# datatypevoid/babble

Measured on AMD Instinct MI355X. Metric: consensus-ordered events/sec at N=256 peers (1 GPU and 8-GPU batched sims), higher is better.
Workload: dtype int32

## Files before the change

### babble_amd/csrc/hgx_api.cpp

```cpp
#include <algorithm>
#include <array>
#include <chrono>
#include <cstdio>
#include <cstring>
#include <mutex>
#include <tuple>
#include <set>
#include <new>
#include <cstdlib>
#include <string>
#include <thread>
#include <vector>

#include "hgx.h"
#include "hgx_bodies.h"
#include "hgx_diff.h"
#include "hgx_engine.h"
#include "hgx_wire_plan.h"

namespace {

struct Block {
    int32_t rr;
    int64_t first;
// ... 2518 lines not shown
    if (x == y) return 1;
    if (!known_div(c, x) || !known_div(c, y)) return 0;
    DeviceGuard dg(c);
    if (ensure_mirror(c) || !same_graph(c, x, y)) return 0;
    std::vector<int32_t> la(c->n), fd(c->n);
    if (c->eng.get_coords(x, la.data(), fd.data()) != hipSuccess) return 0;
    return la[c->creator[(size_t)y] % c->n] >= c->index32[(size_t)y] ? 1 : 0;
}
int32_t hgx_self_ancestor(hgx_ctx* c, int64_t x, int64_t y) {
    if (x == y) return 1;
    if (!c || x < 0 || y < 0 || x >= c->E || y >= c->E) return 0;
    DeviceGuard dg(c);
    if (ensure_mirror(c)) return 0;
    return (c->creator[(size_t)x] == c->creator[(size_t)y] && c->index32[(size_t)x] >= c->index32[(size_t)y]) ? 1 : 0;
}
int32_t hgx_see(hgx_ctx* c, int64_t x, int64_t y) { return hgx_ancestor(c, x, y); }
int32_t hgx_strongly_see(hgx_ctx* c, int64_t x, int64_t y) {
    if (!known_div(c, x) || !known_div(c, y)) return 0;
    DeviceGuard dg(c);
    if (ensure_mirror(c) || !same_graph(c, x, y)) return 0;
    std::vector<int32_t> lx(c->n), fx(c->n), ly(c->n), fy(c->n);
    if (c->eng.get_coords(x, lx.data(), fx.data()) != hipSuccess) return 0;
    if (c->eng.get_coords(y, ly.data(), fy.data()) != hipSuccess) return 0;
    int cnt = 0;
    for (int i = 0; i < c->n; i++) cnt += lx[i] >= fy[i];
    return cnt >= c->sm ? 1 : 0;
}
int64_t hgx_oldest_self_ancestor_to_see(hgx_ctx* c, int64_t x, int64_t y) {
    if (!known_div(c, x) || !known_div(c, y)) return -1;
    DeviceGuard dg(c);
    if (ensure_chains(c) || !same_graph(c, x, y)) return -1;
    std::vector<int32_t> la(c->n), fd(c->n);
    if (c->eng.get_coords(y, la.data(), fd.data()) != hipSuccess) return -1;
    const int cx = c->creator[(size_t)x];
    const int32_t a = fd[cx % c->n];
    if (a <= c->index32[(size_t)x]) return c->chain_gids[cx][(size_t)(a - c->chain_base[cx])];
    return -1;
}
int32_t hgx_round(hgx_ctx* c, int64_t x) {
    if (!c) return -1;
    DeviceGuard dg(c);
    if (ensure_rounds(c)) return -1;
    return round_of(c, x);
}
int32_t hgx_witness(hgx_ctx* c, int64_t x) {
    if (!c) return 0;
    DeviceGuard dg(c);
    if (ensure_rounds(c) || ensure_mirror(c)) return 0;
    return witness_of(c, x);
}

int32_t hgx_phase_times(hgx_ctx* c, double* out, int32_t cap) {
    if (!c || !out) return 0;
    const int32_t m = std::min<int32_t>(cap, 27);
    double v[27] = {c->eng.phase_ms[0], c->eng.phase_ms[1], c->eng.phase_ms[2], c->eng.phase_ms[3],
                    (double)c->eng.la_sweeps, (double)c->eng.R, (double)c->eng.compact,
                    (double)c->eng.la_rows, c->eng.last_rebuild ? 1.0 : 0.0, (double)c->rh.r_lo,
                    c->eng.la_wave_used ? 1.0 : 0.0, (double)c->eng.la_wave_fallbacks,
                    (double)(c->eng.la_wave_used ? c->eng.la_wave_segs : 0), (double)c->eng.round_p_runs,
                    (double)c->eng.round_p_fallbacks, (double)c->eng.round_p_ovf,
                    (double)c->eng.round_p_fail_round, (double)c->eng.round_p_fail_chain,
                    (double)c->eng.round_g_runs, c->eng.la_small_used ? 1.0 : 0.0,
                    c->eng.la_verified ? 1.0 : 0.0, (double)c->eng.sort_seg_runs, (double)c->eng.pipe_used,
                    c->host_ms[0], c->host_ms[1], c->host_ms[2], c->host_ms[3]};
    for (int32_t i = 0; i < m; i++) out[i] = v[i];
    return m;
}

static const char* kKernelNames[hgx::K_NUM] = {"layout", "la_sweep", "fd_build", "round_gather", "round_search",
                                              "fame", "threshold", "round_received", "cts_median", "order_sort"};

int32_t hgx_kernel_stats(hgx_ctx* c, int32_t k, char* name, int32_t name_cap, double* ms, int64_t* launches,
                         double* bytes) {
    if (!c || k < 0 || k >= hgx::K_NUM) return HGX_ERR_INVALID;
    if (name && name_cap > 0) std::snprintf(name, (size_t)name_cap, "%s", kKernelNames[k]);
    const hgx::KernelStat& ks = c->eng.kstat[k];
    if (ms) *ms = (ks.timed > 0 && ks.timed < ks.launches) ? ks.ms * (double)ks.launches / (double)ks.timed : ks.ms;
    if (launches) *launches = c->eng.kstat[k].launches;
    if (bytes) *bytes = c->eng.kstat[k].bytes;
    return HGX_OK;
}

int32_t hgx_reset_stats(hgx_ctx* c) {
    if (!c) return HGX_ERR_INVALID;
    for (auto& s : c->eng.kstat) s = hgx::KernelStat();
    return HGX_OK;
}

int32_t hgx_set_coord_storage(hgx_ctx* c, int32_t mode) {
    if (!c || mode < 0 || mode > 1) return HGX_ERR_INVALID;
    each_shard(c, [&](hgx_ctx* x) { x->eng.force_coord32 = mode == 1; });
    return HGX_OK;
}

int32_t hgx_set_kernel_timing(hgx_ctx* c, int32_t on) {
    if (!c) return HGX_ERR_INVALID;
    each_shard(c, [&](hgx_ctx* x) { x->eng.time_mask = (uint32_t)on; });
    return HGX_OK;
}

int32_t hgx_set_fame_tally(hgx_ctx* c, int32_t mode) {
    if (!c || mode < 0 || mode > 2) return HGX_ERR_INVALID;
    each_shard(c, [&](hgx_ctx* x) { x->eng.fame_tally = mode; });
    return HGX_OK;
}

int32_t hgx_device_alloc(int32_t device, int64_t bytes, void** ptr) {
    if (!ptr || bytes < 0) return HGX_ERR_INVALID;
    *ptr = nullptr;
    int prev = -1;
    (void)hipGetDevice(&prev);
    if (hipSetDevice(device) != hipSuccess) return HGX_ERR_DEVICE;
    const hipError_t e = hipMalloc(ptr, (size_t)std::max<int64_t>(bytes, 1));
    if (prev >= 0 && prev != device) (void)hipSetDevice(prev);
    return e == hipSuccess ? HGX_OK : HGX_ERR_DEVICE;
}

// ... 144 lines not shown
        q->eng.la_segs_override = c->eng.la_segs_override;
        q->eng.la_small_override = c->eng.la_small_override;
        q->eng.round_kernel = c->eng.round_kernel;
        q->eng.round_pb_enabled = c->eng.round_pb_enabled;
        q->eng.sort_seg_enabled = c->eng.sort_seg_enabled;
        q->eng.cts_kernel = c->eng.cts_kernel;
        q->eng.incremental = c->eng.incremental;
        q->grp = nullptr;
        c->peers.push_back(q);
    }
    std::vector<hgx_ctx*> sh{c};
    sh.insert(sh.end(), c->peers.begin(), c->peers.end());
    for (int k = 0; k < W; k++) {
        g->eng[k] = &sh[k]->eng;
        sh[k]->eng.grp = g;
        sh[k]->eng.shard = k;
        sh[k]->shard_rank = k;
        sh[k]->shard_world = W;
        sh[k]->eng.shard_lo = g->c_split[k];
        sh[k]->eng.shard_hi = g->c_split[k + 1];
    }
    return ok(err);
}

int32_t hgx_set_shard_remote(hgx_ctx* c, int32_t on) {
    if (!c || !c->grp || on < 0 || on > 1) return HGX_ERR_INVALID;
    c->grp->force_remote = on != 0;
    return HGX_OK;
}

int32_t hgx_set_round_shards(hgx_ctx* c, int32_t shards) {
    if (!c || shards < 1 || shards > hgx::kMaxShards) return HGX_ERR_INVALID;
    if (shards == (c->grp ? c->grp->W : 1)) return HGX_OK;
    std::vector<int32_t> devs((size_t)shards, c->eng.dev);
    return setup_group(c, shards, devs.data(), nullptr);
}

hgx_ctx* hgx_create_sharded(int32_t n_participants, int64_t capacity_events, int32_t n_shards, const int32_t* devices,
                            hgx_error* err) {
    if (n_shards < 1 || n_shards > hgx::kMaxShards || !devices) {
        set_err(err, HGX_ERR_INVALID, "hgx_create_sharded: 1 to 8 shards, one device ordinal each");
        return nullptr;
    }
    hgx_ctx* c = hgx_create_batch(1, n_participants, capacity_events, devices[0], err);
    if (!c) return nullptr;
    if (setup_group(c, n_shards, devices, err) != HGX_OK) {
        hgx_destroy(c);
        return nullptr;
    }
    return c;
}

int32_t hgx_set_cts_kernel(hgx_ctx* c, int32_t mode) {
    if (!c || mode < 0 || mode > 2) return HGX_ERR_INVALID;
    each_shard(c, [&](hgx_ctx* x) { x->eng.cts_kernel = mode == 0 ? 1 : mode; });
    return HGX_OK;
}

int32_t hgx_set_commit_callback(hgx_ctx* c, hgx_commit_fn fn, void* user) {
    if (!c) return HGX_ERR_INVALID;
    c->commit_fn = fn;
    c->commit_user = user;
    return HGX_OK;
}

int32_t hgx_set_incremental(hgx_ctx* c, int32_t on) {
    if (!c || on < 0 || on > 1) return HGX_ERR_INVALID;
    each_shard(c, [&](hgx_ctx* x) { x->eng.incremental = on != 0; });
    return HGX_OK;
}

int32_t hgx_reserve_rounds(hgx_ctx* c, int32_t rounds) {
    if (!c || rounds < 1 || c->divided) return HGX_ERR_INVALID;
    int32_t rc = HGX_OK;
    each_shard(c, [&](hgx_ctx* x) {
        DeviceGuard dg(x);
        if (x->eng.reserve_rounds(rounds) != hipSuccess) rc = HGX_ERR_DEVICE;
        x->rounds_cached = x->recv_cached = false;
    });
    return rc;
}

}
```

### babble_amd/csrc/hgx_cts.hip

```cpp
#include <hip/hip_runtime.h>

#include <algorithm>
#include <climits>
#include <cstdint>

#include "hgx_device.h"
#include "hgx_kernels.h"

namespace hgx {

constexpr int kCpT = 8;
constexpr int kCpRing = 4;
constexpr int kCpMaxC = 4096;
constexpr int64_t kCtsRedo = (int64_t)0x8000000000000000ull;

struct CtsTileInfo {
    int32_t row[kCpT];
    int64_t ts[kCpT];
    int32_t tc, p0;
};

__device__ __forceinline__ void cp_lds_barrier() { asm volatile("s_waitcnt lgkmcnt(0)\n\ts_barrier" ::: "memory"); }
__device__ __forceinline__ void cp_order() { asm volatile("" ::: "memory"); }

// ... 209 lines not shown
        const int64_t res = (int64_t)(wave_select_kth<CPL>(v, ok, m / 2, whist[wave]) ^ 0x8000000000000000ull);
        if (lane == 0) p_cts[p] = res;
    }
}

template <int NPAD, typename CT>
static bool cts_pipe_launch(hipStream_t s, const DevArrays& a, int c_lo, int c_cnt, int C, int n, int64_t P,
                            int max_cnt) {
    constexpr int LD = kCpT + 1;
    const size_t lds = (((size_t)4 * C + (size_t)8 * c_cnt + 15) & ~(size_t)15) + (size_t)2 * NPAD * LD * 5;
    const void* f = (const void*)k_cts_pipe<NPAD, CT>;
    static int dev_cus[64] = {0};
    int dev = 0;
    if (hipGetDevice(&dev) != hipSuccess || dev < 0 || dev >= 64) return false;
    if (ensure_lds_limit(f, lds) != hipSuccess) return false;
    if (dev_cus[dev] == 0) {
        int cus = 0;
        if (hipDeviceGetAttribute(&cus, hipDeviceAttributeMultiprocessorCount, dev) != hipSuccess || cus <= 0)
            return false;
        dev_cus[dev] = cus;
    }
    int per_cu = 0;
    if (blocks_per_cu(f, 256, lds, &per_cu) != hipSuccess || per_cu < 1) return false;
    const int ntt = (max_cnt + kCpT - 1) / kCpT;
    const int64_t tiles = (int64_t)c_cnt * ntt;
    if (tiles <= 0) return true;
    if (tiles > 0x7FFFFFFF - (int64_t)dev_cus[dev] * per_cu) return false;
    const unsigned grid = (unsigned)std::min<int64_t>(tiles, (int64_t)dev_cus[dev] * per_cu);
    hipLaunchKernelGGL((k_cts_pipe<NPAD, CT>), dim3(grid), dim3(256), lds, s, a.fu, a.rcnt, a.p_rr, a.c_off, a.c_base,
                       a.WLAT, (const CT*)a.FDT, a.p_ts, a.p_cts, C, n, P, c_lo, c_cnt, ntt);
    hipLaunchKernelGGL((k_cts_redo<NPAD, CT>), dim3((max_cnt + 255) / 256, c_cnt), dim3(256), 0, s, a.fu, a.rcnt, a.p_rr,
                       a.c_off, a.c_base, a.WLAT, (const CT*)a.FDT, a.p_ts, a.p_cts, C, n, P, c_lo);
    return true;
}

template <typename CT>
static bool launch_cts_pipe_t(hipStream_t s, const DevArrays& a, int c_lo, int c_cnt, int C, int n, int64_t P,
                              int max_cnt) {
    if (n <= 64) return cts_pipe_launch<64, CT>(s, a, c_lo, c_cnt, C, n, P, max_cnt);
    if (n <= 128) return cts_pipe_launch<128, CT>(s, a, c_lo, c_cnt, C, n, P, max_cnt);
    if (n <= 256) return cts_pipe_launch<256, CT>(s, a, c_lo, c_cnt, C, n, P, max_cnt);
    return cts_pipe_launch<512, CT>(s, a, c_lo, c_cnt, C, n, P, max_cnt);
}

bool cts_pipe_ok(int n, int C) { return n > 32 && n <= 512 && C <= kCpMaxC; }

bool launch_cts_pipe(hipStream_t s, const DevArrays& a, int c_lo, int c_cnt, int C, int n, int64_t P, int max_cnt) {
    if (max_cnt <= 0 || c_cnt <= 0) return true;
    if (!cts_pipe_ok(n, C)) return false;
    return a.compact ? launch_cts_pipe_t<uint16_t>(s, a, c_lo, c_cnt, C, n, P, max_cnt)
                     : launch_cts_pipe_t<int32_t>(s, a, c_lo, c_cnt, C, n, P, max_cnt);
}

}
```

### babble_amd/csrc/hgx_engine.cpp

```cpp
#include "hgx_engine.h"

#include <algorithm>
#include <array>
#include <chrono>
#include <cstdio>
#include <cstdlib>
#include <cstring>
#include <functional>

namespace hgx {

#define HGX_TRY(x)                              \
    do {                                        \
        hipError_t _e = (x);                    \
        if (_e != hipSuccess) return _e;        \
    } while (0)

template <typename T>
hipError_t DBuf<T>::alloc(size_t count) {
    release();
    if (count == 0) count = 1;
    hipError_t e = hipMalloc((void**)&p, count * sizeof(T));
    if (e == hipSuccess) n = count; else p = nullptr;
    return e;
// ... 2019 lines not shown
    return find_order_end(out, nullptr);
}

hipError_t Engine::find_order_begin(const std::vector<uint8_t>& el, const std::vector<uint8_t>& famous,
                                    const std::vector<uint8_t>& ure, int32_t r0, int max_unrecv, OrderHost& out) {
    stage_out.clear();
    pend.clear();
    stage_used = 0;
    out = OrderHost();
    fo_m = 0;
    fo_cnt.assign(C, 0);
    if (R == 0 || E_div == 0 || max_unrecv == 0 || r0 >= R) return hipSuccess;
    DevArrays a = arrays();
    HGX_TRY(hipEventRecord(ph0, stream));
    const size_t o = (size_t)r0 * C;
    HGX_TRY(stage_h2d(elig.p, el.data(), (size_t)G * R));
    HGX_TRY(stage_h2d(fw.p + o, famous.data() + o, (size_t)R * C - o));
    HGX_TRY(stage_h2d(ur_empty.p, ure.data(), (size_t)G));
    HGX_TRY(stage_issue());
    if (WLAT.n < (size_t)R * C * n) {
        const size_t want = (size_t)R * C * n + (size_t)C * n;
        const size_t first = WLAT.n ? 0 : std::min((size_t)r_cap * C * n, (size_t)1 << 28);
        HGX_TRY(WLAT.alloc(std::max(want, std::max(2 * WLAT.n, first))));
        a = arrays();
    }
    kbeg(K_THRESHOLD);
    launch_wla_transpose(stream, a, r0, R, G, C, n);
    launch_threshold(stream, a, r0, R, C, n);
    kend(K_THRESHOLD, 0);
    {
        FillRange fr[2] = {{counters.p, 8, 0}, {rcnt.p, (uint32_t)((size_t)C * 4), 0}};
        launch_fill_many(stream, fr, 2);
        HGX_TRY(hipGetLastError());
    }
    kbeg(K_ROUND_RECEIVED);
    launch_round_received(stream, a, R, C, n, max_unrecv);
    kend(K_ROUND_RECEIVED, 0);
    HGX_TRY(copy_to_pinned(h_small, counters.p, 8));
    HGX_TRY(stage_d2h(fo_cnt.data(), rcnt.p, (size_t)C * 4));
    HGX_TRY(stage_issue());
    HGX_TRY(hipStreamSynchronize(stream));
    stage_flush();
    fo_m = h_small[0];
    out.panic = h_small[1] != 0;
    out.m = fo_m;
    int max_cnt = 0, unrecv = 0;
    for (int c = 0; c < C; c++) unrecv += h_len_div[c] - h_fu[c];
    for (int c = shard_lo; c < shard_hi; c++) max_cnt = std::max(max_cnt, fo_cnt[c]);
    kadd_bytes(K_ROUND_RECEIVED, (double)unrecv * 16);
    if (out.panic || fo_m == 0) {
        fo_m = 0;
        return collect_kernel_times();
    }
    kbeg(K_CTS);
    if (cts_kernel != 2 || !launch_cts_pipe(stream, a, shard_lo, shard_hi - shard_lo, C, n, fd_ld, max_cnt))
        launch_cts(stream, a, shard_lo, shard_hi - shard_lo, C, n, fd_ld, max_cnt);
    int64_t own = 0;
    for (int c = shard_lo; c < shard_hi; c++) own += fo_cnt[c];
    kend(K_CTS, (double)own * (4.0 * n + 8.0 * n));
    return hipSuccess;
}

int64_t Engine::shard_values(int lo, int hi) const {
    int64_t k = 0;
    for (int c = lo; c < hi && c < (int)fo_cnt.size(); c++) k += fo_cnt[c];
    return k;
}

hipError_t Engine::shard_copy(int lo, int hi, void* buf, bool on_device, bool to_buf) {
    const int64_t cnt = shard_values(lo, hi);
    if (cnt == 0) return hipSuccess;
    std::vector<int32_t> offs(C + 1, 0);
    for (int c = lo; c < hi; c++) offs[c + 1] = offs[c] + fo_cnt[c];
    if (sh_off.n < (size_t)C + 1) HGX_TRY(sh_off.alloc((size_t)C + 1));
    HGX_TRY(hipMemcpyAsync(sh_off.p, offs.data(), (size_t)(C + 1) * 4, hipMemcpyHostToDevice, stream));
    int64_t* dev = (int64_t*)buf;
    if (!on_device) {
        if (sh_buf.n < (size_t)cnt) HGX_TRY(sh_buf.alloc((size_t)cnt));
        dev = sh_buf.p;
        if (!to_buf) HGX_TRY(hipMemcpyAsync(dev, buf, (size_t)cnt * 8, hipMemcpyHostToDevice, stream));
    }
    launch_cts_shard_copy(stream, arrays(), lo, hi, sh_off.p, dev, to_buf ? 1 : 0);
    if (!on_device && to_buf) HGX_TRY(hipMemcpyAsync(buf, dev, (size_t)cnt * 8, hipMemcpyDeviceToHost, stream));
    return hipStreamSynchronize(stream);
}

hipError_t Engine::find_order_end(OrderHost& out, int32_t* order_dst) {
    HGX_TRY(payload_wait_S());
    out.blk_cnt.assign((size_t)G * std::max(R, 1), 0);
    out.blk_ntx.assign((size_t)G * std::max(R, 1), 0);
    out.blk_loaded.assign((size_t)G * std::max(R, 1), 0);
    out.blk_nil.assign((size_t)G * std::max(R, 1), 0);
    const int32_t m = fo_m;
    if (m == 0) return hipSuccess;
    fo_m = 0;
    DevArrays a = arrays();
    uint32_t* vals = nullptr;
    const bool small = sort_small_ok(m);
    {
        FillRange fr[5] = {{blk_cnt.p, (uint32_t)((size_t)G * R * 4), 0},
                           {blk_loaded.p, (uint32_t)((size_t)G * R * 4), 0},
                           {blk_ntx.p, (uint32_t)((size_t)G * R * 8), 0},
                           {blk_nil.p, (uint32_t)((size_t)G * R), 0},
                           {val_b.p, (uint32_t)((size_t)m * 4), 0}};
        launch_fill_many(stream, fr, small ? 5 : 4);
        HGX_TRY(hipGetLastError());
    }
    void* dst_dev = nullptr;
    const bool big_dst = order_dst && (size_t)m * 4 > kCopyKernelMax &&
                         hipHostGetDevicePointer(&dst_dev, order_dst, 0) == hipSuccess && dst_dev;
    if (order_dst && !big_dst) (void)hipGetLastError();
// ... 199 lines not shown
```

### babble_amd/csrc/hgx_engine.h

```cpp
#pragma once

#include <hip/hip_runtime.h>

#include <cstdint>
#include <string>
#include <atomic>
#include <condition_variable>
#include <mutex>
#include <thread>
#include <vector>

#include "hgx_kernels.h"

namespace hgx {


constexpr int kStepBatch = 16;
constexpr int kStepBatchSmall = 2;

struct StepGraph {
    hipGraph_t graph = nullptr;
    hipGraphExec_t exec = nullptr;
    std::vector<hipGraphNode_t> nodes;
    std::vector<hipKernelNodeParams> params;
// ... 187 lines not shown
    hipError_t decide_fame_wait();
    hipError_t find_order(const std::vector<uint8_t>& elig, const std::vector<uint8_t>& famous,
                          const std::vector<uint8_t>& ur_empty, int32_t r0, int max_unrecv, OrderHost& out);
    int32_t recv_round_lo(const RoundsHost& rh, int& max_unrecv) const;
    hipError_t find_order_begin(const std::vector<uint8_t>& elig, const std::vector<uint8_t>& famous,
                                const std::vector<uint8_t>& ur_empty, int32_t r0, int max_unrecv, OrderHost& out);
    hipError_t find_order_end(OrderHost& out, int32_t* order_dst = nullptr);
    int64_t shard_values(int lo, int hi) const;
    hipError_t shard_copy(int lo, int hi, void* buf, bool on_device, bool to_buf);
    int shard_lo = 0, shard_hi = 0;
    hipError_t set_roots(const std::vector<int32_t>& round, const std::vector<uint8_t>& y_ext);
    hipError_t set_root_others(const uint8_t* keys32, int64_t count);
    bool others_trust = false;
    bool rooted = false;
    int root_gmax = -1;
    hipError_t round_first_gids(int32_t r0, std::vector<int32_t>& out);
    hipError_t copy_order(int32_t* dst, int64_t first, int64_t count);
    hipError_t sync() { return hipStreamSynchronize(stream); }

    hipError_t reset_received();
    hipError_t reserve_rounds(int32_t rounds);
    hipError_t get_rounds(std::vector<int32_t>& round_by_gid);
    hipError_t get_received(std::vector<int32_t>& rr, std::vector<int64_t>& cts);
    hipError_t get_coords(int64_t gid, int32_t* la, int32_t* fd);

    int n = 0, G = 0, C = 0, sm = 0, nw = 1;
    int64_t cap = 0, E = 0, E_div = 0;
    int64_t Ppos = 0;
    bool incremental = true;
    bool last_rebuild = false;
    int32_t R = 0;
    int la_sweeps = 0;
    int la_kernel = 0;
    bool la_wave_used = false;
    int la_wave_segs = 1;
    int la_segs_override = 0;
    int num_cus = 256;
    static constexpr int kLaMaxSegs = 16;
    static constexpr int kLaHeadRows = 64;
    static constexpr int kLaSegMinRows = 512;
    int64_t la_wave_fallbacks = 0;
    bool la_verified = false;
    bool la_verify_always = false;
    int compact = 0;
    bool force_coord32 = false;
    int64_t la_rows = 0;
    static constexpr int kLaSeg = 16;
    hipStream_t stream = nullptr;
    double phase_ms[4] = {0, 0, 0, 0};
    KernelStat kstat[K_NUM];
    uint32_t time_mask = 0;
    int fame_tally = 0;
    int round_kernel = 0;
    int cts_kernel = 1;
    int64_t round_g_runs = 0;
    ShardGroup* grp = nullptr;
    int shard = 0;
    hipError_t share_round_rows(int32_t r_a, int32_t r_b);
    hipError_t capture_steps(StepGraph& sgr, const RoundArgs& args, int kern, int nb);
    bool la_small_used = false;
    int la_small_override = -1;
    bool sort_seg_enabled = true;
    int64_t sort_seg_runs = 0;
    bool round_pb_enabled = true;
    int64_t round_p_runs = 0, round_p_fallbacks = 0;
    int64_t round_p_ovf = 0;
    int32_t round_p_fail_round = -1, round_p_fail_chain = -1;
    int dev = 0;

   private:
    hipError_t ensure_round_cap(int32_t need);
    hipError_t insert_impl(const InsertIn& in, int64_t count, InsertOut& out, const unsigned long long* fail_sig,
                           int commit_mode = kCommitAll);
    struct WireRun {
        const int32_t* win;
        int64_t slots;
        int64_t *out_sp, *out_op;
    };
    hipError_t insert_bodies_run(const BodiesIn& ev, const std::vector<int64_t>& txi, int64_t count,
                                 const uint8_t* op_id32, uint8_t* out_id32, InsertOut& out, const WireRun* wire);
    hipStream_t stream2 = nullptr;
    void layout_slots(int64_t En, const std::vector<int32_t>& chain_len, std::vector<int32_t>& off) const;
    int rebuild_segments(int64_t En, int coord_compact) const;
    hipStream_t stream_p = nullptr;
    hipEvent_t ev_pc[kPipeMaxPieces + 1] = {}, ev_lay[kPipeMaxPieces] = {}, ev_side[2] = {};
    std::atomic<int> pipe_stage{0};
    std::atomic<int> pipe_stop{0};
    std::thread pipe_thread;
    hipError_t pipe_err = hipSuccess;
    DBuf<int32_t> pipe_buf;
    std::vector<int32_t> pipe_hist, pipe_lim, pipe_off;
    bool pipe_ready = false;
    int64_t pipe_En = 0;
    int pipe_nts = 0, pipe_compact = 0;
    bool pay32 = false;
    bool split32 = false;
    hipEvent_t ev_pay = nullptr;
    hipEvent_t ev_pay_S = nullptr;
    std::atomic<int> pay_stage{0};
    bool pay_S_pending = false;
    bool pay_commit_pending = false;
    int64_t pay_E0 = 0, pay_m = 0;
    bool fame_pending = false;
    bool rows_pending = false;
    size_t rows_n = 0;
    std::thread pay_thread;
    hipError_t pay_err = hipSuccess;
// ... 133 lines not shown
```

### babble_amd/csrc/hgx_kernels.h

```cpp
#pragma once

#include <hip/hip_runtime.h>

#include <cstdint>
#include <functional>
#include <vector>

namespace hgx {

constexpr int32_t kMaxI32 = 2147483647;
constexpr int32_t kWlatNotFamous = -2147483647 - 1;
constexpr int kOpkBits = 21;

struct DevArrays {
    const int32_t *g_creator, *g_index, *g_op, *g_ntx;
    const int64_t* g_ts;
    const uint8_t *g_S, *g_coin, *g_loaded, *g_txnil;
    int32_t *g_rr, *g_pos;
    int64_t* g_ck;
    int64_t* g_cts;
    const int32_t *c_off, *c_len, *c_base;
    int32_t *p_gid, *p_chain, *p_op, *p_opu, *p_round, *p_rr;
    int32_t* p_opk;
    int64_t *p_ts, *p_cts;
// ... 122 lines not shown
                     int32_t stamp, int64_t* usum, int32_t* out, int32_t* out_next, const int32_t* c_old, int64_t u0);
void launch_fd_build(hipStream_t s, const DevArrays& a, int C, int n, int max_len, int64_t P, const int32_t* c_old,
                     int max_new, int d_lo = 0, int d_hi = -1);
void launch_init_new(hipStream_t s, const DevArrays& a, int64_t E0, int64_t m, int n, int64_t P);
void launch_round_gather(hipStream_t s, const DevArrays& a, int r, int C, int n, int64_t P);
void launch_wcoin(hipStream_t s, const DevArrays& a, int r0, int R, int C);
hipError_t launch_round_step(hipStream_t s, const RoundArgs& A, int r, int block_search);
hipError_t launch_round_k(hipStream_t s, const RoundArgs& A, int r);
void launch_round_k_gather(hipStream_t s, const RoundArgs& A, int r);
int round_k_ndw(int n);
bool round_p_ok(int n, int C, int num_cus);
bool round_g_ok(int n, int nw);
hipError_t launch_round_g(hipStream_t s, const RoundArgs& A, int32_t* status, int32_t* fin, int r0, int r_end);
constexpr int kRoundPBufs = 4;
constexpr int kRoundPShift = 2;
constexpr int kMaxShards = 8;
struct RoundPWindows {
    int nwin = 0;
    uint32_t remote = 0;
    uint32_t* FD8p[kMaxShards] = {};
    uint64_t* gran[kMaxShards] = {};
    int32_t* st[kMaxShards] = {};
    const void* FDT[kMaxShards] = {};
    int32_t c_split[kMaxShards + 1] = {};
};
hipError_t launch_xchg_floor(hipStream_t s, int C, int n, int rounds, uint32_t* rows, uint64_t* gran, int32_t* st);
hipError_t launch_round_p(hipStream_t s, const RoundArgs& A, uint32_t* FD8p, uint64_t* gran, int32_t* status,
                          int32_t* fin, int r0, int r_end, int init, int num_cus, int c_lo = 0, int c_hi = -1,
                          const RoundPWindows* win_dev = nullptr, int nwin = 1);
void launch_round_p_tail(hipStream_t s, const RoundArgs& A, const int32_t* fin, int r_last);
void launch_round_p_post(hipStream_t s, const RoundArgs& A, int r_lo, int r_hi);
bool round_pb_ok(int n, int G);
hipError_t launch_round_pb(hipStream_t s, const RoundArgs& A, uint32_t* FD8p, uint64_t* gran, int32_t* status,
                           int32_t* fin, const int32_t* amap, int na, int r0, int r_end, int num_cus, bool init);
void launch_round_pb_silent(hipStream_t s, const RoundArgs& A, int r_lo, int r_hi);
void launch_root_floor(hipStream_t s, const DevArrays& a, const int32_t* root_round, int32_t* gfl, int32_t* gB,
                       int gmax, int C, int n, int max_len);
void launch_round_first_gid(hipStream_t s, const DevArrays& a, int r0, int R, int C, int32_t* first);
void launch_last_round(hipStream_t s, int rs, int R, int G, int C, int n, const uint8_t* wstat, int32_t* lr);
void step_prof_dump();
void round_k_prof_dump();
void round_p_prof_dump();
void round_pb_prof_dump();
void round_g_prof_dump();
void launch_fame(hipStream_t s, const DevArrays& a, int r0, int R, int C, int n, int nw, int sm, int G, int tally);
void launch_wla_transpose(hipStream_t s, const DevArrays& a, int r0, int R, int G, int C, int n);
void launch_threshold(hipStream_t s, const DevArrays& a, int r0, int R, int C, int n);
void launch_round_received(hipStream_t s, const DevArrays& a, int R, int C, int n, int max_unrecv);
void launch_fu_advance(hipStream_t s, const DevArrays& a, int C);
void launch_fu_count(hipStream_t s, const DevArrays& a, int64_t E);
void launch_cts(hipStream_t s, const DevArrays& a, int c_lo, int c_cnt, int C, int n, int64_t P, int max_cnt);
bool cts_pipe_ok(int n, int C);
bool launch_cts_pipe(hipStream_t s, const DevArrays& a, int c_lo, int c_cnt, int C, int n, int64_t P, int max_cnt);
void launch_cts_shard_copy(hipStream_t s, const DevArrays& a, int lo, int hi, const int32_t* offs, int64_t* buf,
                           int to_buf);
void launch_minmax(hipStream_t s, const DevArrays& a, int32_t m);
void launch_sort(hipStream_t s, const DevArrays& a, int32_t m, int64_t cmin, int cts_bits, int R, int n,
                 int seg_bits, uint32_t** final_vals, uint64_t** final_keys);
int seg_sort_cap();
void launch_seg_count(hipStream_t s, const DevArrays& a, int32_t m, int R, int n, int nseg, uint32_t* segc,
                      unsigned long long* max_out);
hipError_t launch_sort_seg(hipStream_t s, const DevArrays& a, int32_t m, int64_t cmin, int cts_bits, int R, int n, int nseg,
                     uint32_t* segoff, uint32_t* segcur, int max_seg, uint32_t** final_vals, uint64_t** final_keys,
                     const std::vector<int>* cuts = nullptr,
                     const std::function<hipError_t(int)>& after_part = nullptr);
bool sort_small_ok(int32_t m);
void launch_sort_small(hipStream_t s, const DevArrays& a, int32_t m, int n, uint32_t** final_vals);
void launch_finish_order(hipStream_t s, const DevArrays& a, int32_t m, const uint32_t* vals, int R, int n);
void launch_gather_i32(hipStream_t s, int64_t E, const int32_t* src, const int32_t* g_pos, int32_t* dst);

size_t p256_table_bytes(int nk);
void launch_p256_tables(hipStream_t s, int nk, const uint8_t* keys65, uint32_t* tab, uint8_t* valid);
void launch_p256_verify(hipStream_t s, int64_t count, int nk, const int32_t* key_idx, const uint8_t* dig,
                        const uint8_t* r, const uint8_t* sg, const uint32_t* tab, const uint8_t* valid, uint8_t* out);

void launch_insert_claim(hipStream_t s, int64_t m, int64_t E0, int64_t cap, int C, const InsertIn& in,
                         const InsertState& st);
void launch_insert_check(hipStream_t s, int64_t m, int64_t E0, int64_t cap, int C, int n, const InsertIn& in,
                         const InsertState& st);
constexpr int kCommitAll = 0, kCommitStructure = 1, kCommitPayload = 2;
void launch_insert_commit(hipStream_t s, int64_t m, const unsigned long long* fail, const unsigned long long* fail_sig,
                          int64_t E0, int n, const InsertIn& in, const InsertState& st, int mode);
constexpr int kPipeMaxPieces = 8;
void launch_pipe_hist(hipStream_t s, int pieces, const int64_t* cut, int C, const int32_t* creator, int32_t* hist);
void launch_pipe_insert(hipStream_t s, int64_t m, int64_t E0, int64_t cap, int C, int n, const InsertIn& in,
                        const InsertState& st, int32_t* gate);
void launch_ts_to_pos(hipStream_t s, int64_t E0, int64_t m, const int32_t* g_pos, const int64_t* g_ts, int64_t* p_ts);
void launch_insert_unclaim(hipStream_t s, int64_t m, const unsigned long long* fail, const unsigned long long* fail_sig,
                           int64_t E0, int64_t cap, int C, const InsertIn& in, const InsertState& st);
bool launch_insert_fused(hipStream_t s, int64_t m, const unsigned long long* fail_sig, int64_t E0, int64_t cap, int C,
                         int n, const InsertIn& in, const InsertState& st, int mode);
void launch_insert_sig_first(hipStream_t s, int64_t m, int C, const int32_t* creator, const uint8_t* vout,
                             unsigned long long* fail);
void launch_unpack_packed(hipStream_t s, int64_t m, int64_t E0, const uint16_t* c16, const uint16_t* spb,
                          const uint16_t* opb, int64_t n_exc, const int64_t* exc_pos, const int32_t* exc_sp,
                          const int32_t* exc_op, int32_t* cr, int32_t* sp, int32_t* op);

void launch_scan_u32(hipStream_t s, uint32_t* buf, int64_t total, uint32_t* part);

struct PruneArgs {
    int64_t E, n_kept;
    int C;
    const int32_t *g_creator, *g_index, *g_sp, *g_op, *g_ntx;
    const int64_t* g_ts;
    const uint8_t *g_S, *g_id, *g_txnil;
    const int32_t* cut;
// ... 48 lines not shown
```

### babble_amd/hashgraph.py

```python
from __future__ import annotations

import ctypes as C
import os
from typing import List, Optional, Sequence

import numpy as np

from . import _lib
from ._lib import HgxError, hgx_error, hgx_events, ptr

UNKNOWN_PARENT = -2


def compact_columns(t) -> dict:
    ntx = np.where(np.asarray(t.txnil) != 0, -1, np.asarray(t.ntx)).astype(np.int32)
    return dict(creator=np.ascontiguousarray(t.creator, np.int32), index=np.ascontiguousarray(t.index, np.int32),
                sp=np.ascontiguousarray(t.sp, np.int32), op=np.ascontiguousarray(t.op, np.int32),
                ts=np.ascontiguousarray(t.ts, np.int64),
                coin=np.ascontiguousarray(np.asarray(t.hash)[:, 16] != 0, np.uint8),
                s=np.ascontiguousarray(t.s, np.uint8), ntx=ntx)


class HostBuffer:

# ... 708 lines not shown
        return bool(self.L.hgx_strongly_see(self.ctx, x, y))

    def OldestSelfAncestorToSee(self, x: int, y: int) -> int:
        return int(self.L.hgx_oldest_self_ancestor_to_see(self.ctx, x, y))

    def Round(self, x: int) -> int:
        return int(self.L.hgx_round(self.ctx, x))

    def Witness(self, x: int) -> bool:
        return bool(self.L.hgx_witness(self.ctx, x))

    def coords(self, x: int):
        la = np.zeros(self.n, np.int32)
        fd = np.zeros(self.n, np.int32)
        rc = self.L.hgx_get_coords(self.ctx, x, ptr(la), ptr(fd))
        if rc:
            raise HgxError(rc, "hgx_get_coords failed")
        return la, fd

    def num_events(self) -> int:
        return int(self.L.hgx_num_events(self.ctx))

    def rounds(self):
        E = self.num_events()
        rnd = np.zeros(max(E, 1), np.int32)
        wit = np.zeros(max(E, 1), np.int8)
        fam = np.zeros(max(E, 1), np.int8)
        if E:
            rc = self.L.hgx_get_rounds(self.ctx, 0, E, ptr(rnd), ptr(wit), ptr(fam))
            if rc:
                raise HgxError(rc, "hgx_get_rounds failed")
        return rnd[:E], wit[:E], fam[:E]

    def received(self):
        E = self.num_events()
        rr = np.zeros(max(E, 1), np.int32)
        cts = np.zeros(max(E, 1), np.int64)
        if E:
            rc = self.L.hgx_get_received(self.ctx, 0, E, ptr(rr), ptr(cts))
            if rc:
                raise HgxError(rc, "hgx_get_received failed")
        return rr[:E], cts[:E]

    def results(self, graph: int = 0) -> dict:
        rnd, wit, fam = self.rounds()
        rr, cts = self.received()
        return dict(round=rnd, witness=wit, famous=fam, rr=rr, cts=np.where(rr >= 0, cts, 0),
                    order=self.ConsensusEvents(graph), last_round=self.LastRound(graph),
                    undecided=self.UndecidedRounds(graph), lcr=self.LastConsensusRound(graph),
                    lcre=self.LastCommitedRoundEvents(graph), consensus_tx=self.ConsensusTransactions(graph),
                    pending_loaded=self.PendingLoadedEvents(graph), blocks=self.Blocks(graph))

    def phase_times(self):
        out = np.zeros(27, np.float64)
        self.L.hgx_phase_times(self.ctx, ptr(out), 27)
        return dict(coords_ms=out[0], rounds_ms=out[1], fame_ms=out[2], order_ms=out[3],
                    la_sweeps=int(out[4]), rounds=int(out[5]), compact=int(out[6]),
                    la_rows=int(out[7]), rebuild=int(out[8]), r_lo=int(out[9]),
                    la_wave=int(out[10]), la_wave_fallbacks=int(out[11]), la_wave_segs=int(out[12]),
                    round_p_runs=int(out[13]), round_p_fallbacks=int(out[14]), round_p_ovf=int(out[15]),
                    round_p_fail_round=int(out[16]), round_p_fail_chain=int(out[17]),
                    round_g_runs=int(out[18]), la_small=int(out[19]), la_verify=int(out[20]),
                    sort_seg=int(out[21]), ingest_pieces=int(out[22]),
                    host_rounds_ms=out[23], host_fame_ms=out[24], host_order_ms=out[25],
                    payload_end_ms=out[26])

    def set_ingest_pipeline(self, pieces, min_events=4_000_000):
        if self.L.hgx_set_ingest_pipeline(self.ctx, int(pieces), int(min_events)) != 0:
            raise ValueError(f"invalid ingest pipeline {pieces}, {min_events}")

    def set_fame_tally(self, mode):
        m = {"popc": 0, "vote": 1, "mfma": 2}[mode] if isinstance(mode, str) else int(mode)
        if self.L.hgx_set_fame_tally(self.ctx, m) != 0:
            raise ValueError(f"invalid fame tally {mode}")

    def set_la_kernel(self, mode):
        m = {"wave": 0, "sweep": 1, "ring": 1025, "wave+verify": 1026}[mode] if isinstance(mode, str) else int(mode)
        if self.L.hgx_set_la_kernel(self.ctx, m) != 0:
            raise ValueError(f"invalid lastAncestors kernel {mode}")

    def set_round_kernel(self, mode):
        m = ({"auto": 0, "block": 1, "candidate": 2, "persistent": 3, "graph": 4, "auto-steps": 5}[mode]
             if isinstance(mode, str) else int(mode))
        if self.L.hgx_set_round_kernel(self.ctx, m) != 0:
            raise ValueError(f"invalid round kernel {mode}")

    def set_sort_kernel(self, mode):
        m = {"auto": 0, "radix": 1}[mode] if isinstance(mode, str) else int(mode)
        if self.L.hgx_set_sort_kernel(self.ctx, m) != 0:
            raise ValueError(f"invalid sort kernel {mode}")

    def set_round_shards(self, shards: int):
        if self.L.hgx_set_round_shards(self.ctx, int(shards)) != 0:
            raise ValueError(f"invalid shard count {shards} (an empty context, 1..8 shards, "
                             f"GPU_MAX_HW_QUEUES >= shards + 2 for shards sharing a device)")

    def set_shard_remote(self, on: bool = True):
        if self.L.hgx_set_shard_remote(self.ctx, 1 if on else 0) != 0:
            raise ValueError("hgx_set_shard_remote: not a chain-sharded context")

    def set_cts_kernel(self, mode):
        m = {"auto": 0, "tile": 1, "pipe": 2}[mode] if isinstance(mode, str) else int(mode)
        if self.L.hgx_set_cts_kernel(self.ctx, m) != 0:
            raise ValueError(f"invalid timestamp kernel {mode}")

    def set_incremental(self, on: bool):
        if self.L.hgx_set_incremental(self.ctx, 1 if on else 0) != 0:
            raise ValueError("invalid schedule")

    def reserve_rounds(self, rounds: int):
        if self.L.hgx_reserve_rounds(self.ctx, int(rounds)) != 0:
            raise ValueError("hgx_reserve_rounds failed")

    def set_coord_storage(self, mode):
        if self.L.hgx_set_coord_storage(self.ctx, int(mode)) != 0:
            raise ValueError(f"invalid coordinate storage mode {mode}")

    def kernel_stats(self):
        res = {}
        for k in range(10):
            name = C.create_string_buffer(32)
            ms, launches, nbytes = C.c_double(), C.c_int64(), C.c_double()
            if self.L.hgx_kernel_stats(self.ctx, k, name, 32, C.byref(ms), C.byref(launches), C.byref(nbytes)):
                break
            res[name.value.decode()] = dict(ms=ms.value, launches=launches.value, bytes=nbytes.value)
        return res

    KERNELS = ("layout", "la_sweep", "fd_build", "round_gather", "round_search", "fame", "threshold",
               "round_received", "cts_median", "order_sort")

    def set_kernel_timing(self, which=True):
        if which is True:
            mask = -1
        elif not which:
            mask = 0
        else:
            mask = 1 << self.KERNELS.index(which)
        self.L.hgx_set_kernel_timing(self.ctx, mask)

    def reset_stats(self):
        self.L.hgx_reset_stats(self.ctx)


class DeviceBuffer:

    def __init__(self, a: np.ndarray, device: int = 0):
        self.L = _lib.lib()
        self.device = device
        a = np.ascontiguousarray(a)
        self.nbytes = a.nbytes
        self.p = C.c_void_p()
        if self.L.hgx_device_alloc(device, max(1, a.nbytes), C.byref(self.p)) != 0:
            raise HgxError(200, "hgx_device_alloc failed")
        if a.nbytes and self.L.hgx_device_copy(device, self.p, ptr(a), a.nbytes, 1) != 0:
            self.close()
# ... 152 lines not shown
```

Before: 263.0 million.

## Add row-tiled consensus-timestamp median kernel and auto-select it for large batches

Adds a new k_cts_row kernel that computes consensus timestamps per tile of 64 events. It stages witness-lattice rows in LDS, stores 32-bit timestamp deltas transposed in shared memory, and has each wave select the median through a shared histogram, falling back to 64-bit values on overflow. The default cts_kernel becomes auto (0), which picks the row kernel when n is in (32,256] and there are at least eight tiles of events per chain; otherwise it uses the existing tile or pipe kernels. The aim is more data reuse and fewer global gathers in the median step, at the cost of heavy LDS use and per-event fallback paths.

```diff
diff --git a/babble_amd/csrc/hgx_api.cpp b/babble_amd/csrc/hgx_api.cpp
--- a/babble_amd/csrc/hgx_api.cpp
+++ b/babble_amd/csrc/hgx_api.cpp
@@ -2594,8 +2594,8 @@
 
 int32_t hgx_phase_times(hgx_ctx* c, double* out, int32_t cap) {
     if (!c || !out) return 0;
-    const int32_t m = std::min<int32_t>(cap, 27);
-    double v[27] = {c->eng.phase_ms[0], c->eng.phase_ms[1], c->eng.phase_ms[2], c->eng.phase_ms[3],
+    const int32_t m = std::min<int32_t>(cap, 28);
+    double v[28] = {c->eng.phase_ms[0], c->eng.phase_ms[1], c->eng.phase_ms[2], c->eng.phase_ms[3],
                     (double)c->eng.la_sweeps, (double)c->eng.R, (double)c->eng.compact,
                     (double)c->eng.la_rows, c->eng.last_rebuild ? 1.0 : 0.0, (double)c->rh.r_lo,
                     c->eng.la_wave_used ? 1.0 : 0.0, (double)c->eng.la_wave_fallbacks,
@@ -2604,7 +2604,7 @@
                     (double)c->eng.round_p_fail_round, (double)c->eng.round_p_fail_chain,
                     (double)c->eng.round_g_runs, c->eng.la_small_used ? 1.0 : 0.0,
                     c->eng.la_verified ? 1.0 : 0.0, (double)c->eng.sort_seg_runs, (double)c->eng.pipe_used,
-                    c->host_ms[0], c->host_ms[1], c->host_ms[2], c->host_ms[3]};
+                    c->host_ms[0], c->host_ms[1], c->host_ms[2], c->host_ms[3], (double)c->eng.cts_row_runs};
     for (int32_t i = 0; i < m; i++) out[i] = v[i];
     return m;
 }
@@ -2855,8 +2855,8 @@
 }
 
 int32_t hgx_set_cts_kernel(hgx_ctx* c, int32_t mode) {
-    if (!c || mode < 0 || mode > 2) return HGX_ERR_INVALID;
-    each_shard(c, [&](hgx_ctx* x) { x->eng.cts_kernel = mode == 0 ? 1 : mode; });
+    if (!c || mode < 0 || mode > 4) return HGX_ERR_INVALID;
+    each_shard(c, [&](hgx_ctx* x) { x->eng.cts_kernel = mode; });
     return HGX_OK;
 }
 
diff --git a/babble_amd/csrc/hgx_cts.hip b/babble_amd/csrc/hgx_cts.hip
--- a/babble_amd/csrc/hgx_cts.hip
+++ b/babble_amd/csrc/hgx_cts.hip
@@ -285,4 +285,202 @@
                      : launch_cts_pipe_t<int32_t>(s, a, c_lo, c_cnt, C, n, P, max_cnt);
 }
 
-}
+constexpr int kRowKMax = 8;
+constexpr int kRowTP = 64;
+constexpr int kRowD = 16;
+constexpr int row_waves(int npad) { return npad >= 128 ? 8 : 4; }
+
+template <int NPAD, typename CT, int TP, int DREQ, int NW>
+__global__ void __launch_bounds__(64 * NW) k_cts_row(const int32_t* __restrict__ fu, const int32_t* __restrict__ rcnt,
+                                                 const int32_t* __restrict__ p_rr, const int32_t* __restrict__ c_off,
+                                                 const int32_t* __restrict__ c_base, const int32_t* __restrict__ WLAT,
+                                                 const CT* __restrict__ FDT, const int64_t* __restrict__ p_ts,
+                                                 int64_t* __restrict__ p_cts, int C, int n, int64_t Pcap, int c_lo,
+                                                 int c_cnt, int R, int K) {
+    static_assert(TP == 64, "k_cts_row: a wave's lanes are the block's events");
+    constexpr int LD = TP + 1;
+    constexpr int CPL = NPAD / 64;
+    constexpr int CW = NPAD / NW;
+    constexpr int NI = CW;
+    constexpr int D = DREQ < NI ? DREQ : NI;
+    constexpr int NB = NI / D;
+    constexpr int MB = NPAD / 8;
+    static_assert(NI % D == 0 && NI % 8 == 0 && NI <= 64, "k_cts_row: batches and membership bytes");
+    constexpr int RG = 64 * NW / NPAD;
+    constexpr int KL = kRowKMax / RG;
+    static_assert(RG >= 1 && kRowKMax % RG == 0, "k_cts_row: staging loads");
+    extern __shared__ __attribute__((aligned(16))) uint32_t vals[];
+    int32_t* wl = (int32_t*)(vals + NPAD * LD);
+    __shared__ uint8_t mem[TP][MB];
+    __shared__ int32_t e_row[TP];
+    __shared__ int64_t e_ts[TP];
+    __shared__ int32_t e_ovf[TP];
+    __shared__ uint32_t s_min[NW];
+    const int cl = (int)(blockIdx.x % (unsigned)c_cnt), tt = (int)(blockIdx.x / (unsigned)c_cnt);
+    const int tc = c_lo + cl;
+    const int f0 = fu[tc], co = c_off[tc];
+    const int64_t q0 = (int64_t)co + f0, pend = q0 + rcnt[tc];
+    const int64_t ps = (int64_t)co + (f0 & ~31) + (int64_t)tt * TP;
+    if ((ps > q0 ? ps : q0) >= pend) return;
+    const int lane = lane_id(), wave = __builtin_amdgcn_readfirstlane((int)(threadIdx.x >> 6));
+    const int e = lane;
+    const int64_t p = ps + e;
+    const bool ev = p >= q0 && p < pend;
+    const int64_t pl = ev ? p : (ps > q0 ? ps : q0);
+    const int i = p_rr[pl];
+    const int64_t base = p_ts[pl];
+    const int g = tc / n, gb = g * n;
+    const int j = c_base[tc] + (int)(pl - co);
+    const bool evi = ev && i >= 0;
+    const int wc0 = wave * CW;
+    uint32_t* whist = vals + NPAD * LD + 256 * wave;
+    auto chain = [&](int k) { const int c = wc0 + k; return c < n ? c : 0; };
+    auto load_fd = [&](int b, CT (&fd)[D]) {
+#pragma unroll
+        for (int u = 0; u < D; u++) fd[u] = FDT[(size_t)chain(b * D + u) * Pcap + pl];
+    };
+    CT fd[2][D];
+    load_fd(0, fd[0]);
+    const int kc = wc0 + lane < n && lane < CW ? wc0 + lane : 0;
+    const int32_t kdv = c_off[gb + kc] - c_base[gb + kc];
+    const uint32_t wmin = wave_reduce_min_u32(evi ? (uint32_t)i : 0x7fffffffu);
+    if (lane == 0) s_min[wave] = wmin;
+    if (threadIdx.x < TP) {
+        e_row[e] = evi ? i : -1;
+        e_ts[e] = base;
+        e_ovf[e] = 0;
+    }
+    cp_lds_barrier();
+    uint32_t bmin = s_min[0];
+#pragma unroll
+    for (int w = 1; w < NW; w++) bmin = min(bmin, s_min[w]);
+    const int imin = bmin == 0x7fffffffu ? 0 : (int)bmin;
+    int32_t st[KL];
+    const int sw = (int)threadIdx.x % NPAD, srow = (int)threadIdx.x / NPAD;
+#pragma unroll
+    for (int q = 0; q < KL; q++)
+        st[q] = WLAT[((size_t)min(imin + min(q * RG + srow, K - 1), R - 1) * C + tc) * n + min(sw, n - 1)];
+    int64_t x[2][D];
+    auto gather = [&](int b, const CT (&f)[D], int64_t (&xo)[D]) {
+#pragma unroll
+        for (int u = 0; u < D; u++) {
+            const int k = b * D + u;
+            const int32_t kd = __builtin_amdgcn_readlane(kdv, k);
+            const int32_t fv = Coord<CT>::fd(f[u]);
+            xo[u] = p_ts[fv != kMaxI32 ? kd + fv : 0];
+        }
+    };
+    uint64_t ovm = 0;
+    if (NB > 1) load_fd(1, fd[1]);
+    cp_order();
+    gather(0, fd[0], x[0]);
+    cp_order();
+#pragma unroll
+    for (int b = 0; b < NB; b++) {
+        if (b + 2 < NB) load_fd(b + 2, fd[b & 1]);
+        cp_order();
+        if (b + 1 < NB) gather(b + 1, fd[(b + 1) & 1], x[(b + 1) & 1]);
+        cp_order();
+#pragma unroll
+        for (int u = 0; u < D; u++) {
+            const int k = b * D + u;
+            const int64_t dlt = x[b & 1][u] - base;
+            ovm |= (uint64_t)(dlt < INT32_MIN || dlt > INT32_MAX) << k;
+            vals[(wc0 + k) * LD + e] = (uint32_t)(int32_t)dlt ^ 0x80000000u;
+        }
+        cp_order();
+    }
+    const int WS = n + 1;
+#pragma unroll
+    for (int q = 0; q < KL; q++)
+        if (q * RG + srow < K && sw < n) wl[(q * RG + srow) * WS + sw] = st[q];
+    __syncthreads();
+    {
+        uint64_t okm = 0;
+        if (!evi || i - imin < K) {
+            const int32_t* row = wl + (evi ? i - imin : 0) * WS;
+#pragma unroll
+            for (int k = 0; k < NI; k++) okm |= (uint64_t)(row[chain(k)] >= j) << k;
+        } else {
+            const int32_t* __restrict__ row = WLAT + ((size_t)i * C + tc) * n;
+#pragma unroll
+            for (int k = 0; k < NI; k++) okm |= (uint64_t)(row[chain(k)] >= j) << k;
+        }
+        const int live = n - wc0;
+        if (live < NI) okm &= live > 0 ? ((uint64_t)1 << live) - 1 : 0;
+        if (!evi) okm = 0;
+#pragma unroll
+        for (int q = 0; q < NI / 8; q++) mem[e][wc0 / 8 + q] = (uint8_t)(okm >> (8 * q));
+        if (ovm & okm) e_ovf[e] = 1;
+    }
+    __syncthreads();
+    for (int e2 = wave; e2 < TP; e2 += NW) {
+        if (e_row[e2] < 0) continue;
+        bool ok[CPL];
+        int m = 0;
+#pragma unroll
+        for (int q = 0; q < CPL; q++) {
+            const int c = lane + 64 * q;
+            ok[q] = (mem[e2][c >> 3] >> (c & 7)) & 1u;
+            m += __popcll(__ballot(ok[q]));
+        }
+        int64_t res;
+        if (!e_ovf[e2]) {
+            uint32_t v[CPL];
+#pragma unroll
+            for (int q = 0; q < CPL; q++) v[q] = vals[(lane + 64 * q) * LD + e2];
+            const uint32_t u = wave_select_kth32<CPL>(v, ok, m / 2, whist);
+            res = e_ts[e2] + (int64_t)(int32_t)(u ^ 0x80000000u);
+        } else {
+            uint64_t v[CPL];
+#pragma unroll
+            for (int q = 0; q < CPL; q++) {
+                const int c = lane + 64 * q;
+                int64_t x = 0;
+                if (ok[q]) x = p_ts[c_off[gb + c] - c_base[gb + c] + Coord<CT>::fd(FDT[(size_t)c * Pcap + ps + e2])];
+                v[q] = (uint64_t)x ^ 0x8000000000000000ull;
+            }
+            res = (int64_t)(wave_select_kth<CPL>(v, ok, m / 2, whist) ^ 0x8000000000000000ull);
+        }
+        if (lane == 0) p_cts[ps + e2] = res;
+    }
+}
+
+template <int NPAD, typename CT>
+static bool cts_row_launch(hipStream_t s, const DevArrays& a, int c_lo, int c_cnt, int C, int n, int64_t P,
+                           int max_cnt, int R, int k_rows) {
+    constexpr int TP = kRowTP, NW = row_waves(NPAD);
+    constexpr size_t kStatic = (size_t)TP * (NPAD / 8) + (size_t)TP * 16 + 4 * NW;
+    const size_t fixed = (size_t)NPAD * (TP + 1) * 4, row = (size_t)(n + 1) * 4;
+    const int room = (int)(((size_t)79 * 1024 - kStatic - fixed) / row);
+    const int K = k_rows > 0 ? std::min(k_rows, kRowKMax) : std::max(1, std::min(room, kRowKMax));
+    const size_t lds = fixed + std::max((size_t)K * row, (size_t)NW * 1024);
+    const void* f = (const void*)k_cts_row<NPAD, CT, TP, kRowD, NW>;
+    if (ensure_lds_limit(f, lds) != hipSuccess) return false;
+    const int64_t blocks = (int64_t)c_cnt * ((max_cnt + 31 + TP - 1) / TP);
+    if (blocks > 0x7FFFFFFF) return false;
+    hipLaunchKernelGGL((k_cts_row<NPAD, CT, TP, kRowD, NW>), dim3((unsigned)blocks), dim3(64 * NW), lds, s, a.fu, a.rcnt, a.p_rr,
+                       a.c_off, a.c_base, a.WLAT, (const CT*)a.FDT, a.p_ts, a.p_cts, C, n, P, c_lo, c_cnt, R, K);
+    return true;
+}
+
+template <typename CT>
+static bool launch_cts_row_t(hipStream_t s, const DevArrays& a, int c_lo, int c_cnt, int C, int n, int64_t P,
+                             int max_cnt, int R, int k_rows) {
+    if (n <= 64) return cts_row_launch<64, CT>(s, a, c_lo, c_cnt, C, n, P, max_cnt, R, k_rows);
+    if (n <= 128) return cts_row_launch<128, CT>(s, a, c_lo, c_cnt, C, n, P, max_cnt, R, k_rows);
+    return cts_row_launch<256, CT>(s, a, c_lo, c_cnt, C, n, P, max_cnt, R, k_rows);
+}
+
+bool cts_row_ok(int n) { return n > 32 && n <= 256; }
+int cts_row_tile() { return kRowTP; }
+
+bool launch_cts_row(hipStream_t s, const DevArrays& a, int c_lo, int c_cnt, int C, int n, int64_t P, int max_cnt,
+                    int R, int k_rows) {
+    if (max_cnt <= 0 || c_cnt <= 0) return true;
+    if (!cts_row_ok(n) || R <= 0) return false;
+    return a.compact ? launch_cts_row_t<uint16_t>(s, a, c_lo, c_cnt, C, n, P, max_cnt, R, k_rows)
+                     : launch_cts_row_t<int32_t>(s, a, c_lo, c_cnt, C, n, P, max_cnt, R, k_rows);
+}
+
+}
diff --git a/babble_amd/csrc/hgx_engine.cpp b/babble_amd/csrc/hgx_engine.cpp
--- a/babble_amd/csrc/hgx_engine.cpp
+++ b/babble_amd/csrc/hgx_engine.cpp
@@ -2095,11 +2095,17 @@
         fo_m = 0;
         return collect_kernel_times();
     }
-    kbeg(K_CTS);
-    if (cts_kernel != 2 || !launch_cts_pipe(stream, a, shard_lo, shard_hi - shard_lo, C, n, fd_ld, max_cnt))
-        launch_cts(stream, a, shard_lo, shard_hi - shard_lo, C, n, fd_ld, max_cnt);
     int64_t own = 0;
     for (int c = shard_lo; c < shard_hi; c++) own += fo_cnt[c];
+    const int c_cnt = shard_hi - shard_lo;
+    constexpr int kCtsRowMinTiles = 8;
+    const bool row = cts_row_ok(n) &&
+        (cts_kernel >= 3 || (cts_kernel == 0 && own >= (int64_t)kCtsRowMinTiles * cts_row_tile() * c_cnt));
+    kbeg(K_CTS);
+    if (row && launch_cts_row(stream, a, shard_lo, c_cnt, C, n, fd_ld, max_cnt, R, cts_kernel == 4 ? 1 : 0))
+        cts_row_runs++;
+    else if (cts_kernel != 2 || !launch_cts_pipe(stream, a, shard_lo, c_cnt, C, n, fd_ld, max_cnt))
+        launch_cts(stream, a, shard_lo, c_cnt, C, n, fd_ld, max_cnt);
     kend(K_CTS, (double)own * (4.0 * n + 8.0 * n));
     return hipSuccess;
 }
diff --git a/babble_amd/csrc/hgx_engine.h b/babble_amd/csrc/hgx_engine.h
--- a/babble_amd/csrc/hgx_engine.h
+++ b/babble_amd/csrc/hgx_engine.h
@@ -263,7 +263,8 @@
     uint32_t time_mask = 0;
     int fame_tally = 0;
     int round_kernel = 0;
-    int cts_kernel = 1;
+    int cts_kernel = 0;
+    int64_t cts_row_runs = 0;
     int64_t round_g_runs = 0;
     ShardGroup* grp = nullptr;
     int shard = 0;
diff --git a/babble_amd/csrc/hgx_kernels.h b/babble_amd/csrc/hgx_kernels.h
--- a/babble_amd/csrc/hgx_kernels.h
+++ b/babble_amd/csrc/hgx_kernels.h
@@ -198,6 +198,10 @@
 void launch_cts(hipStream_t s, const DevArrays& a, int c_lo, int c_cnt, int C, int n, int64_t P, int max_cnt);
 bool cts_pipe_ok(int n, int C);
 bool launch_cts_pipe(hipStream_t s, const DevArrays& a, int c_lo, int c_cnt, int C, int n, int64_t P, int max_cnt);
+bool cts_row_ok(int n);
+int cts_row_tile();
+bool launch_cts_row(hipStream_t s, const DevArrays& a, int c_lo, int c_cnt, int C, int n, int64_t P, int max_cnt,
+                    int R, int k_rows);
 void launch_cts_shard_copy(hipStream_t s, const DevArrays& a, int lo, int hi, const int32_t* offs, int64_t* buf,
                            int to_buf);
 void launch_minmax(hipStream_t s, const DevArrays& a, int32_t m);
diff --git a/babble_amd/hashgraph.py b/babble_amd/hashgraph.py
--- a/babble_amd/hashgraph.py
+++ b/babble_amd/hashgraph.py
@@ -784,8 +784,8 @@
                     pending_loaded=self.PendingLoadedEvents(graph), blocks=self.Blocks(graph))
 
     def phase_times(self):
-        out = np.zeros(27, np.float64)
-        self.L.hgx_phase_times(self.ctx, ptr(out), 27)
+        out = np.zeros(28, np.float64)
+        self.L.hgx_phase_times(self.ctx, ptr(out), 28)
         return dict(coords_ms=out[0], rounds_ms=out[1], fame_ms=out[2], order_ms=out[3],
                     la_sweeps=int(out[4]), rounds=int(out[5]), compact=int(out[6]),
                     la_rows=int(out[7]), rebuild=int(out[8]), r_lo=int(out[9]),
@@ -795,7 +795,7 @@
                     round_g_runs=int(out[18]), la_small=int(out[19]), la_verify=int(out[20]),
                     sort_seg=int(out[21]), ingest_pieces=int(out[22]),
                     host_rounds_ms=out[23], host_fame_ms=out[24], host_order_ms=out[25],
-                    payload_end_ms=out[26])
+                    payload_end_ms=out[26], cts_row=int(out[27]))
 
     def set_ingest_pipeline(self, pieces, min_events=4_000_000):
         if self.L.hgx_set_ingest_pipeline(self.ctx, int(pieces), int(min_events)) != 0:
@@ -832,7 +832,7 @@
             raise ValueError("hgx_set_shard_remote: not a chain-sharded context")
 
     def set_cts_kernel(self, mode):
-        m = {"auto": 0, "tile": 1, "pipe": 2}[mode] if isinstance(mode, str) else int(mode)
+        m = {"auto": 0, "tile": 1, "pipe": 2, "row": 3, "row1": 4}[mode] if isinstance(mode, str) else int(mode)
         if self.L.hgx_set_cts_kernel(self.ctx, m) != 0:
             raise ValueError(f"invalid timestamp kernel {mode}")
 
```

After: 267.2 million, median of 6. +1.6%, better.
